# zhen6618/EPRecon

Measured on AMD Instinct MI355X. Metric: fragments_per_sec, higher is better.
Workload: dtype f32

## Files before the change

### eprecon_amd/_lib.py

```python
import ctypes
import os

import numpy as np
import torch

_HERE = os.path.dirname(os.path.abspath(__file__))
LIB_PATH = os.environ.get("EPRECON_LIB_PATH") or os.path.join(_HERE, "libeprecon_hip.so")

_c = ctypes
_vp, _i, _i64, _f, _sz = _c.c_void_p, _c.c_int, _c.c_int64, _c.c_float, _c.c_size_t

SIGNATURES = {
    "eprecon_abi_version": (_i, []),
    "eprecon_build_arch": (_c.c_char_p, []),
    "eprecon_count_mailbox": (_i, []),
    "eprecon_mailbox_acquire": (_i, [_i, _vp]),
    "eprecon_mailbox_wait": (_i, [_vp, _i64, _vp]),
    "eprecon_mailbox_release": (_i, [_vp]),
    "eprecon_mailbox_free_slots": (_i, []),
    "eprecon_back_project_workspace_bytes": (_sz, [_i64, _i, _i, _i, _i, _i, _i]),
    "eprecon_back_project_async": (_i, [_vp, _i64, _vp, _i, _f, _vp, _i, _vp, _i, _i, _i, _i, _i, _i,
                                        _vp, _vp, _vp, _vp, _vp, _vp, _vp, _vp, _sz, _vp]),
    "eprecon_back_project_call_async": (_i, [_vp, _vp]),
    "eprecon_back_project_call": (_i, [_vp, _i, _vp, _vp]),
    "eprecon_back_project_prepare_levels_async": (_i, [_vp, _i, _vp]),
    "eprecon_back_project_workspace_maps_offset": (_sz, [_i64, _i]),
    "eprecon_bp_levels": (_i, []),
    "eprecon_init_glue": (_i, []),
    "eprecon_profile_gather_kernel": (_c.c_char_p, []),
    "eprecon_hash_capacity": (_c.c_uint32, [_i64]),
    "eprecon_hash_table_bytes": (_sz, [_c.c_uint32]),
    "eprecon_hash_build_async": (_i, [_vp, _i64, _i, _vp, _c.c_uint32, _vp]),
    "eprecon_hash_build_dn_async": (_i, [_vp, _i64, _vp, _i, _vp, _c.c_uint32, _vp]),
    "eprecon_hash_query_async": (_i, [_vp, _c.c_uint32, _vp, _i64, _i, _vp, _vp]),
    "eprecon_hash_status": (_i, [_vp, _vp]),
    "eprecon_unique_workspace_bytes": (_sz, [_i64]),
    "eprecon_unique_coords_async": (_i, [_vp, _i64, _i, _vp, _c.c_uint32, _vp, _vp, _vp, _vp, _sz, _vp]),
    "eprecon_unique_coords_dn_async": (_i, [_vp, _i64, _vp, _i, _vp, _c.c_uint32, _vp, _vp, _vp, _vp, _sz, _vp]),
    "eprecon_unique_hierarchy_dn_async": (_i, [_vp, _i64, _vp, _i, _vp, _vp, _vp, _vp, _vp, _vp, _sz, _vp]),
    "eprecon_point_quantize_dn_async": (_i, [_vp, _i64, _vp, _f, _vp, _vp, _vp]),
    "eprecon_spvcnn_points_dn_async": (_i, [_vp, _i64, _vp, _i, _i, _vp, _i, _f, _vp, _f, _vp, _vp, _vp, _vp, _vp, _vp]),
    "eprecon_gru_stage_capacity": (_i64, [_vp, _i64, _i]),
# ... 244 lines not shown


class ViewsDesc(ctypes.Structure):
    _fields_ = [("src", (ctypes.c_void_p * 16) * 3), ("dst", ctypes.c_void_p * 3), ("channels", ctypes.c_int32 * 3),
                ("hw", ctypes.c_int32 * 3), ("levels", ctypes.c_int32), ("n_views", ctypes.c_int32)]


class BpCall(ctypes.Structure):
    _fields_ = [("coords", ctypes.c_void_p), ("n", ctypes.c_int64), ("origin", ctypes.c_void_p), ("batch", ctypes.c_int32),
                ("voxel_size", ctypes.c_float), ("feats", ctypes.c_void_p), ("feats_layout", ctypes.c_int32),
                ("krcam", ctypes.c_void_p), ("n_views", ctypes.c_int32), ("channels", ctypes.c_int32), ("height", ctypes.c_int32),
                ("width", ctypes.c_int32), ("min_view", ctypes.c_int32), ("mode", ctypes.c_int32), ("count", ctypes.c_void_p),
                ("n_valid_dev", ctypes.c_void_p), ("workspace", ctypes.c_void_p), ("workspace_bytes", ctypes.c_size_t),
                ("phase", ctypes.c_int32), ("out_feats", ctypes.c_void_p), ("out_mean", ctypes.c_void_p),
                ("out_coords", ctypes.c_void_p), ("out_grid", ctypes.c_void_p), ("out_mask", ctypes.c_void_p),
                ("rank", ctypes.c_void_p), ("counts_host", ctypes.c_void_p), ("counts_seq", ctypes.c_uint32)]


class MailboxSlot(ctypes.Structure):
    _fields_ = [("payload_dev", ctypes.c_void_p), ("payload_host", ctypes.c_void_p), ("seq", ctypes.c_uint32),
                ("index", ctypes.c_int32), ("words", ctypes.c_int32), ("armed", ctypes.c_int32)]


class AdamSegment(ctypes.Structure):
    _fields_ = [("param", ctypes.c_void_p), ("grad", ctypes.c_void_p), ("exp_avg", ctypes.c_void_p),
                ("exp_avg_sq", ctypes.c_void_p)]


class AdamChunk(ctypes.Structure):
    _fields_ = [("segment", ctypes.c_int32), ("start", ctypes.c_int32), ("count", ctypes.c_int32), ("flags", ctypes.c_int32)]

# ... 302 lines not shown
```

### eprecon_amd/back_project.py

```python
import ctypes

import torch
import torch.nn as nn

from . import _lib

MODE_MEAN, MODE_MEAN_DEPTH, MODE_VARIANCE = 0, 1, 2
LAYOUT_NCHW, LAYOUT_NHWC = 0, 1


def mark_dense(coords, dims, interval, batch=1):
    coords._eprecon_dense = (tuple(int(d) for d in dims), int(interval), int(batch))
    return coords


def dense_rank_buffer(coords, dims, interval):
    tag = getattr(coords, "_eprecon_dense", None)
    want = (tuple(int(d) for d in dims), int(interval), 1)
    if tag != want or not coords.is_cuda or coords.shape[0] != want[0][0] * want[0][1] * want[0][2]:
        return None
    if not _lib.load().eprecon_init_glue():
        return None
    return torch.empty(coords.shape[0] + 1, dtype=torch.int32, device=coords.device)

# ... 126 lines not shown
        self._slots = [hd.mailbox for hd in handles]
        self._read = None if all(m is not None for m in self._slots) else _lib.PinnedRead(handles[0].n_valid_all)

    def results(self):
        if self._host is None and self._read is None:
            _lib.count_host_read()
            self._host = [None] * (self._offsets[-1] + 1 + self._pends[-1]._batch)
            for m, p, o in zip(self._slots, self._pends, self._offsets):
                self._host[o:o + 1 + p._batch] = m.wait()
        elif self._host is None:
            self._host = self._read.result()
        return [p.result_from(self._host[o:o + 1 + p._batch]) for p, o in zip(self._pends, self._offsets)]


def prepare_levels_async(levels, stream=None):
    lib = _lib.load()
    if not 1 <= len(levels) <= 4:
        raise _lib.EpreconError("prepare_levels_async takes one to four levels")
    dev = levels[0][3].device
    rows = []
    for lv in levels:
        coords, origin, voxel_size, feats, krcam, min_view = lv[:6]
        mode = lv[6] if len(lv) > 6 else MODE_MEAN
        shape = tuple(int(x) for x in feats.shape)
        feats_c, layout = _prep_feats(feats)
        inputs = None if coords is None else _prep_inputs(coords, origin, krcam, shape[0], shape[1], dev)
        rows.append((shape, feats_c, layout, inputs, float(voxel_size), int(min_view), mode))
    n_valid_all = torch.empty((sum(1 + r[0][1] for r in rows if r[3] is not None),), dtype=torch.int32, device=dev)
    descs = (_lib.BpCall * len(rows))()
    listed = [r for r in rows if r[3] is not None]
# ... 9 lines not shown
        _call(inputs, feats_c, shape, layout, voxel_size, min_view, mode, {"count": count}, n_valid_dev, ws, d=d)
        nhwc = feats_c
        if layout == LAYOUT_NCHW:
            o = lib.eprecon_back_project_workspace_maps_offset(n, b)
            nhwc = ws[o:o + 4 * v * b * c * h * w].view(torch.float32).view(v, b, h, w, c).permute(0, 1, 4, 2, 3)
        if inputs is None:
            handles.append(PreparedMaps(nhwc, (ws, feats_c), stream))
            continue
        mb = next(slots)
        if mb is not None:
            d.counts_host, d.counts_seq = mb.payload_dev, mb.seq
        hd = CountedBackProject(shape, inputs + (voxel_size, min_view, mode), d, count, n_valid_dev, ws, stream, mailbox=mb)
        hd.nhwc, hd.feats, hd.n_valid_all, hd.n_valid_off = nhwc, feats_c, n_valid_all, off
        handles.append(hd)
        off += 1 + b

    def queue():
        _lib.check(lib.eprecon_back_project_prepare_levels_async(ctypes.byref(descs), len(rows), _lib.current_stream()),
                   "eprecon_back_project_prepare_levels_async")
        for hd in handles:
            if getattr(hd, "mailbox", None) is not None:
                hd.mailbox.queued(hd.n_valid_dev)
    if stream is None:
        queue()
    else:
        stream.wait_stream(torch.cuda.current_stream(dev))
        with torch.cuda.stream(stream):
            queue()
    return handles


def run_async(coords, origin, voxel_size, feats, krcam, min_view, mode=MODE_MEAN, min_valid_per_batch=1,
              want_grid=False, want_mean=False, hold_read=False, extra_words=0, rank_out=None, counted=None):
    lib = _lib.load()
    dev = feats.device
    shape = v, b, c, h, w = tuple(feats.shape)
    inputs = _prep_inputs(coords, origin, krcam, v, b, dev)
    n = coords.shape[0]
    feats_c, layout = _prep_feats(feats)
    t = _alloc_outputs(n, v, c, mode, want_grid, want_mean, dev, count=None if counted is None else counted.count)
    if counted is not None:
        assert layout == LAYOUT_NHWC and counted.shape == shape and not extra_words
        assert counted.inputs[3:] == (float(voxel_size), int(min_view), mode) and counted.count.shape[0] == n
        inputs, n_valid_dev, ws = counted.inputs[:3], counted.n_valid_dev, counted.ws
        if counted.stream is not None:
            torch.cuda.current_stream(dev).wait_stream(counted.stream)
    else:
        n_valid_dev = torch.empty((1 + b + int(extra_words),), dtype=torch.int32, device=dev)
        ws = _lib.workspace(lib.eprecon_back_project_workspace_bytes(n, b, v, c, h, w, layout), dev)
    mb, early = (counted.mailbox, counted.early) if counted is not None else (None, False)
    if mb is None and not hold_read and n > 0:
        mb = _lib.mailbox_read(1 + b)
    if counted is not None:
        call = _lib.BpCall.from_buffer_copy(counted.call)
        call.feats, call.feats_layout = _lib.ptr(feats_c), layout
        _set_outputs(call, t, rank_out, phase=2)
    else:
        call = _call(inputs, feats_c, shape, layout, voxel_size, min_view, mode, t, n_valid_dev, ws, rank_out)
    call.counts_host, call.counts_seq = (mb.payload_dev, mb.seq) if mb is not None and not early else (None, 0)
    _lib.check(lib.eprecon_back_project_call_async(ctypes.byref(call), _lib.current_stream()), "eprecon_back_project_call_async")
    if mb is not None and not early:
        mb.queued(n_valid_dev)
    read = None if hold_read else mb if mb is not None else _lib.PinnedRead(n_valid_dev[:1 + b])
    t["_keep"] = (*inputs, feats_c, n_valid_dev, ws if counted is not None else None)
    pend = PendingBackProject(t, n, v, c, b, int(min_valid_per_batch), read, want_grid, want_mean)
    pend.n_valid_dev, pend.coords_all = n_valid_dev, t["coords"]
    return pend


def run(coords, origin, voxel_size, feats, krcam, min_view, mode=MODE_MEAN, min_valid_per_batch=1,
        want_grid=False, want_mean=False, rank_out=None):
    lib = _lib.load()
    dev = feats.device
    shape = v, b, c, h, w = tuple(feats.shape)
# ... 92 lines not shown
```

### eprecon_amd/csrc/back_project.hip

```cpp
#include <stdlib.h>

#include "back_project_gather.hpp"

namespace {

constexpr int kFoldCapDefault = 6144;

size_t gather_lds_bytes(bool mlp, int vox, int V, int B)
{
    const size_t nP = ((size_t)V * B * 12 + 3) & ~(size_t)3;
    return (size_t)vox * V * (mlp ? 12 : 8) + nP * 4 + (size_t)vox * (mlp ? 3 : 5) * 4 + (size_t)(256 / kWave) * 4 * 3;
}

template <int VOX, int MODE>
int launch_gather(const BpParams &p, bool mlp, hipStream_t st)
{
    const size_t lds = gather_lds_bytes(mlp, VOX, p.V, p.batch);
    const dim3 grid(p.ntile), block(256);
    if (p.C % 4 != 0) {
        hipLaunchKernelGGL((bp_gather_kernel<VOX, MODE, 1, 0>), grid, block, lds, st, p);
    } else {
        pick<6, 8, 10, 20, 0>(p.C / 4, [&](auto qt) {
            constexpr int QT = decltype(qt)::value;
            if (mlp) hipLaunchKernelGGL((bp_gather_mlp_kernel<VOX, MODE, QT, 1>), grid, block, lds, st, p);
            else hipLaunchKernelGGL((bp_gather_kernel<VOX, MODE, 4, QT>), grid, block, lds, st, p);
            return 0;
        });
    }
    EP_LAUNCH_CHECK();
    return EPRECON_OK;
}

struct BpCarve {
    size_t rows, maps, end;
// ... 24 lines not shown
    if (!a.workspace || (!a.feats && !(listed && !rows && nhwc))) return EPRECON_ERR_ARG;
    if (listed && (!a.origin || !a.krcam || !a.n_valid_dev)) return EPRECON_ERR_ARG;
    if (listed && a.n > 0 && (!a.coords || !a.count || (rows && (!a.out_feats || !a.out_coords)))) return EPRECON_ERR_ARG;
    if (a.counts_host && (!listed || a.n == 0 || a.counts_seq == 0 || 1 + a.batch > EPRECON_MAILBOX_WORDS)) return EPRECON_ERR_ARG;
    if ((size_t)a.n_views * a.batch * 12 * sizeof(float) > 32 * 1024) return EPRECON_ERR_UNSUPPORTED;
    if (a.workspace_bytes < eprecon_back_project_workspace_bytes(a.n, a.batch, a.n_views, a.channels, a.height, a.width,
                                                                 a.feats_layout))
        return EPRECON_ERR_WORKSPACE;
    if ((size_t)a.n_views * a.batch * a.channels * a.height * a.width > 0x7fffffffull) return EPRECON_ERR_UNSUPPORTED;
    return EPRECON_OK;
}

struct BpPlan {
    bool nchw, chain4, clear_in_relayout, mlp;
    int vox, ntile, nblk_count;
    size_t lds_relayout, lds_count;
    int32_t *tile_sums, *blk_batch;
    float *nhwc;
    BpParams p;
};

BpPlan bp_plan(const eprecon_bp_call &a)
{
    BpPlan pl;
    const int64_t n = a.n;
    pl.nchw = a.feats_layout == EPRECON_LAYOUT_NCHW;
    int fold_cap = kFoldCapDefault;
    if (const char *e = getenv("EPRECON_BP_FOLD"); e && e[0]) {
        const long v = strtol(e, nullptr, 10);
        fold_cap = v <= 0 ? 0 : (v > 0x7fffffffL ? 0x7fffffff : (int)v);
// ... 16 lines not shown
    p.min_view = a.min_view; p.out_feats = a.out_feats; p.out_mean = a.out_mean; p.out_coords = a.out_coords;
    p.count = a.count; p.out_grid = a.out_grid; p.out_mask = a.out_mask; p.n_valid_dev = a.n_valid_dev;
    p.block_offsets = pl.tile_sums;
    p.rank = a.phase == EPRECON_BP_COUNT ? nullptr : a.rank;
    p.counts_host = a.counts_host; p.counts_seq = a.counts_seq;
    p.xcd_slabs = ep::switch_off("EPRECON_BP_XCD_SLABS") ? 0 : 1;
    pl.mlp = p.C % 4 == 0 && p.Cs % 4 == 0 && p.V <= 32 && (size_t)p.V * p.batch * p.H * p.W * p.Cs * 4 < 0x7fff0000ull &&
             gather_lds_bytes(true, 256, p.V, p.batch) <= dynamic_lds_limit();

    pl.vox = n >= 512 * 1024 ? 256 : (n >= 48 * 1024 ? 64 : 16);
    if (pl.vox == 256 && !pl.mlp && gather_lds_bytes(false, 256, a.n_views, a.batch) > dynamic_lds_limit()) pl.vox = 64;
    pl.ntile = (int)ep::ceil_div(n, pl.vox);
    pl.nblk_count = (int)ep::ceil_div(n, 256);
    p.fold = (!pl.chain4 && pl.ntile <= fold_cap) ? 1 : 0;
    p.ntile = pl.ntile; p.blk_batch = pl.blk_batch; p.nblk_count = pl.nblk_count;
    return pl;
}

int bp_clear_counters(const eprecon_bp_call &a, hipStream_t st)
{
    EP_HIP_CHECK(hipMemsetAsync(a.n_valid_dev, 0, sizeof(int32_t) * (size_t)(1 + a.batch), st));
    return EPRECON_OK;
}

int bp_launch_scan(const BpPlan &pl, hipStream_t st, bool write_back = true)
{
    hipLaunchKernelGGL(bp_scan_kernel, dim3(1), dim3(1024), 0, st, pl.tile_sums, pl.ntile, pl.p.n_valid_dev,
                       (const int32_t *)pl.blk_batch, pl.nblk_count, pl.p.batch, write_back ? 1 : 0, pl.p.counts_host,
                       pl.p.counts_seq);
    EP_LAUNCH_CHECK();
// ... 33 lines not shown
    EP_LAUNCH_CHECK();
    if (!p.fold) return bp_launch_scan(pl, st);
    return early_publish && p.counts_host ? bp_launch_scan(pl, st, false) : EPRECON_OK;
}

template <int VOX>
int bp_queue_gather(const eprecon_bp_call &a, const BpPlan &pl, hipStream_t st)
{
    if (a.n == 0) {
        if (a.rank) EP_HIP_CHECK(hipMemsetAsync(a.rank, 0, sizeof(int32_t), st));
        return EPRECON_OK;
    }
    int rc = ep::profile_bracket_begin(st);
    if (rc != EPRECON_OK) return rc;
    rc = pick<EPRECON_BP_MEAN, EPRECON_BP_MEAN_DEPTH, EPRECON_BP_VARIANCE>(
        a.mode, [&](auto mode) { return launch_gather<VOX, decltype(mode)::value>(pl.p, pl.mlp, st); });
    if (rc != EPRECON_OK) return rc;
    rc = ep::profile_bracket_end(st, pl.mlp ? "bp_gather_mlp_kernel" : "bp_gather_kernel");
    if (rc != EPRECON_OK) return rc;
    if (a.mode == EPRECON_BP_MEAN_DEPTH) {
        hipLaunchKernelGGL(bp_depth_norm_kernel, dim3(a.batch), dim3(1024), 0, st, a.out_feats, a.channels + 1, a.n_valid_dev);
        EP_LAUNCH_CHECK();
    }
    return EPRECON_OK;
}

int bp_queue(const eprecon_bp_call &a, const BpPlan &pl, hipStream_t st, bool early_publish = false)
{
    return pick<256, 64, 16>(pl.vox, [&](auto vox) {
        constexpr int VOX = decltype(vox)::value;
        const int rc = a.phase != EPRECON_BP_GATHER ? bp_queue_count<VOX>(a, pl, st, early_publish) : EPRECON_OK;
// ... 72 lines not shown
        d.end = cursor;
    }
    if (cursor > 0) {
        hipLaunchKernelGGL(bp_prepare_levels_kernel, dim3((unsigned)cursor), dim3(256), lds, st, t);
        EP_LAUNCH_CHECK();
    }
    for (int l = 0; l < n_levels; ++l) {
        if (listed[l] && calls[l].n > 0 && !plans[l].p.fold) {
            const int rc = bp_launch_scan(plans[l], st);
            if (rc != EPRECON_OK) return rc;
        }
    }
    return EPRECON_OK;
}

}

extern "C" {

size_t eprecon_back_project_workspace_bytes(int64_t n, int batch, int n_views, int channels,
                                            int height, int width, int feats_layout)
{
    const size_t map_bytes =
        feats_layout == EPRECON_LAYOUT_NCHW ? (size_t)n_views * batch * channels * height * width * sizeof(float) : 0;
    return bp_carve(n > 0 ? n : 1, batch > 0 ? batch : 1, map_bytes).end + 256;
}

size_t eprecon_back_project_workspace_maps_offset(int64_t n, int batch) { return bp_carve(n, batch, 0).maps; }

int eprecon_nchw_to_nhwc_async(const float *in, float *out, int maps, int channels, int hw,
                               void *stream)
{
    if (!in || !out || maps <= 0 || channels <= 0 || hw <= 0) return EPRECON_ERR_ARG;
// ... 59 lines not shown
```

### eprecon_amd/csrc/back_project_gather.hpp

```cpp
#pragma once
#include "back_project_count.hpp"

namespace {


struct TileBase {
    int base, n_valid;
};

__device__ __forceinline__ bool tile_base_all(const BpParams &p, int lb)
{
    return p.out_grid != nullptr || p.out_mask != nullptr || lb == p.ntile - 1;
}

__device__ __forceinline__ void tile_base_partials(const BpParams &p, int lb, int *sFold)
{
    constexpr int BLOCK = 256;
    const int tid = threadIdx.x, lane = tid & (kWave - 1), wid = tid / kWave;
    const int end = tile_base_all(p, lb) ? p.ntile : lb;
    int acc = 0, tot = 0;
#pragma unroll 4
    for (int t = tid; t < end; t += BLOCK) {
        const int x = p.block_offsets[t];
        tot += x;
// ... 37 lines not shown
                if (tid == 0) {
                    int t = 0;
                    for (int w = 0; w < NW; ++w) t += sFold[w];
                    p.n_valid_dev[1 + b] = t;
                }
            }
        }
        if (tid == 0 && p.counts_host) mailbox_publish(p.counts_host, p.counts_seq, p.n_valid_dev, 1 + p.batch);
    }
    return r;
}

__device__ __forceinline__ void gather_rank_store(const BpParams &p, int lb, int e, bool mine, bool valid, int orow)
{
    if (mine) p.rank[e] = valid ? orow : -1;
    if (lb == (int)gridDim.x - 1 && threadIdx.x == 0) p.rank[p.n] = 0;
}


template <int VOX, int MODE, int VEC, int QT>
__global__ __launch_bounds__(256) void bp_gather_kernel(BpParams p)
{
    extern __shared__ __attribute__((aligned(16))) char smem[];
    constexpr int BLOCK = 256;
    float2 *sPix = reinterpret_cast<float2 *>(smem);
    float *sP = reinterpret_cast<float *>(sPix + VOX * p.V);
    const int nP = (p.V * p.batch * 12 + 3) & ~3;
    uint32_t *sVis = reinterpret_cast<uint32_t *>(sP + nP);
    float *sDen = reinterpret_cast<float *>(sVis + VOX);
    int *sBatch = reinterpret_cast<int *>(sDen + VOX);
    int *sSlot = sBatch + VOX;
// ... 136 lines not shown
#pragma unroll
        for (int u = 0; u < U; ++u) {
            const float wx1 = wxy[u].x, wy1 = wxy[u].y;
            const float wx0 = 1.0f - wx1, wy0 = 1.0f - wy1;
            const float w00 = wx0 * wy0, w10 = wx1 * wy0, w01 = wx0 * wy1, w11 = wx1 * wy1;
            float4 r;
#define EP_TAP(k) fmaf(__uint_as_float(d[u].k), w11, fmaf(__uint_as_float(c[u].k), w01, fmaf(__uint_as_float(b[u].k), w10, __uint_as_float(a[u].k) * w00)))
            r.x = EP_TAP(x); r.y = EP_TAP(y); r.z = EP_TAP(z); r.w = EP_TAP(w);
#undef EP_TAP
            if (on[u]) f(r);
        }
    }
}

template <int VOX, int MODE, int QT, int U>
__global__ __launch_bounds__(256) void bp_gather_mlp_kernel(BpParams p)
{
    extern __shared__ __attribute__((aligned(16))) char smem[];
    constexpr int BLOCK = 256;
    constexpr int VPT = BLOCK / VOX;
    float2 *sWxy = reinterpret_cast<float2 *>(smem);
    int *sOff = reinterpret_cast<int *>(sWxy + VOX * p.V);
    float *sP = reinterpret_cast<float *>(sOff + VOX * p.V);
    const int nP = (p.V * p.batch * 12 + 3) & ~3;
    uint32_t *sVis = reinterpret_cast<uint32_t *>(sP + nP);
    int *sSlot = reinterpret_cast<int *>(sVis + VOX);
    int *sOut = sSlot + VOX;
    int *sWave = sOut + VOX;
    int *sFold = sWave + BLOCK / kWave;

    const int tid = threadIdx.x;
    const int lb = p.xcd_slabs ? xcd_remap(blockIdx.x, gridDim.x) : (int)blockIdx.x;
    stage_matrices(sP, p.krcam, p.V * p.batch, tid, BLOCK);
    if (VPT > 1 && tid < VOX) sVis[tid] = 0;
    if (p.fold) tile_base_partials(p, lb, sFold);
    __syncthreads();

    const float wm1 = (float)(p.W - 1), hm1 = (float)(p.H - 1);
    const float kx = 2.0f / wm1, ky = 2.0f / hm1;
    const int map_elems = p.H * p.W * p.Cs;
    const int vx = tid % VOX;
    const int e = lb * VOX + vx;
    int4 c = make_int4(-1, 0, 0, 0);
    if (e < p.n) c = reinterpret_cast<const int4 *>(p.coords)[e];
    const bool in_batch = c.x >= 0 && c.x < p.batch;
    uint32_t vis = 0;
    if (in_batch) {
        float X, Y, Z;
// ... 67 lines not shown
            visit_visible_samples<U>(rsrc, offRow, wxyRow, vm, q * 16, s10, s01, s11, [&](const float4 &f) {
                const float dx = f.x - mean.x, dy = f.y - mean.y, dz = f.z - mean.z, dw = f.w - mean.w;
                sq.x = fmaf(dx, dx, sq.x); sq.y = fmaf(dy, dy, sq.y); sq.z = fmaf(dz, dz, sq.z); sq.w = fmaf(dw, dw, sq.w);
            });
            *reinterpret_cast<float4 *>(dst) = make_float4(__fdiv_rn(sq.x, den), __fdiv_rn(sq.y, den),
                                                           __fdiv_rn(sq.z, den), __fdiv_rn(sq.w, den));
            if (p.out_mean) *reinterpret_cast<float4 *>(p.out_mean + (size_t)orow * p.C + q * 4) = mean;
        } else if (MODE == EPRECON_BP_MEAN_DEPTH) {
            dst[0] = mean.x; dst[1] = mean.y; dst[2] = mean.z; dst[3] = mean.w;
        } else {
            *reinterpret_cast<float4 *>(dst) = mean;
        }
    }
}

__global__ __launch_bounds__(1024) void bp_depth_norm_kernel(float *out_feats, int cout,
                                                             const int32_t *n_valid_dev)
{
    __shared__ float sRed[1024 / kWave];
    const int b = blockIdx.x, tid = threadIdx.x, lane = tid & (kWave - 1), wid = tid / kWave;
    int start = 0;
    for (int k = 0; k < b; ++k) start += n_valid_dev[1 + k];
    const int len = n_valid_dev[1 + b];
    float *d = out_feats + (size_t)start * cout + (cout - 1);

    auto block_sum = [&](float x) -> float {
#pragma unroll
        for (int s = kWave / 2; s > 0; s >>= 1) x += __shfl_xor(x, s);
        __syncthreads();
        if (lane == 0) sRed[wid] = x;
// ... 27 lines not shown
```

### eprecon_amd/csrc/common.hpp

```cpp
#pragma once

#include <hip/hip_runtime.h>
#include <stdint.h>
#include <stdlib.h>

#include <type_traits>

#include "../../include/eprecon_hip.h"

#define EP_HIP_CHECK(expr)                                            \
    do {                                                              \
        hipError_t e_ = (expr);                                       \
        if (e_ != hipSuccess) return EPRECON_ERR_HIP_BASE - (int)e_;  \
    } while (0)
#define EP_LAUNCH_CHECK() EP_HIP_CHECK(hipGetLastError())

namespace ep {

constexpr int kWave = 64;
constexpr int kXcd = 8;

static inline size_t align_up(size_t x, size_t a) { return (x + a - 1) / a * a; }
static inline int64_t ceil_div(int64_t a, int64_t b) { return (a + b - 1) / b; }

inline bool switch_off(const char *name)
{
    const char *e = getenv(name);
    return e && e[0] == '0';
}
inline bool switch_on(const char *name)
{
    const char *e = getenv(name);
    return e && e[0] == '1';
}

// ... 6 lines not shown

static inline size_t dynamic_lds_limit()
{
    static const size_t limit = [] {
        int dev = 0, v = 0;
        if (hipGetDevice(&dev) != hipSuccess ||
            hipDeviceGetAttribute(&v, hipDeviceAttributeMaxSharedMemoryPerBlock, dev) != hipSuccess || v <= 0)
            v = 64 * 1024;
        return (size_t)(v < 64 * 1024 ? v : 64 * 1024);
    }();
    return limit;
}

__device__ __forceinline__ int xcd_remap(int hw_bid, int nblk)
{
    const int q = nblk / kXcd, r = nblk % kXcd;
    const int xcd = hw_bid % kXcd, k = hw_bid / kXcd;
    const int start = xcd < r ? xcd * (q + 1) : r * (q + 1) + (xcd - r) * q;
    return start + k;
}

__device__ __forceinline__ void mailbox_publish(int32_t *payload, uint32_t seq, const int32_t *values, int n)
{
    for (int i = 0; i < n; ++i) payload[i] = values[i];
    __threadfence_system();
    __hip_atomic_store(reinterpret_cast<uint32_t *>(payload) - 1, seq, __ATOMIC_RELEASE, __HIP_MEMORY_SCOPE_SYSTEM);
}

template <int BLOCK>
__device__ __forceinline__ int block_exclusive_rank(bool pred, int *wave_counts, int &block_total)
{
    const unsigned long long m = __ballot(pred);
    const int lane = threadIdx.x & (kWave - 1);
    const int wid = threadIdx.x / kWave;
// ... 36 lines not shown
```

### eprecon_amd/fragment_step.py

```python
import os

import torch

from . import _lib
from . import back_project as BP
from . import grid_ops as GO
from . import synthetic as S
from .config import CH_IMG, CH_INIT_DOWN, N_VIEWS
from .occupancy_initialization import Occupancy_Initialization

LEVELS = [("bp24", 2, 4, 2), ("bp48", 1, 2, 0), ("bp96", 0, 1, 0)]


class Cfg2Step:
    def __init__(self, seed=0, device=None, height=480, width=640, n_vox=(96, 96, 96)):
        self.device = device or torch.device("cuda")
        self.seed = seed
        self.window = S.make_window(seed=seed, width=width, height=height, n_vox=n_vox)
        self.shapes = S.pyramid_shapes(height, width)
        dev = self.device
        t = lambda a: torch.from_numpy(a).to(dev)
        self.origin = t(self.window["vol_origin_partial"][None].copy())
        self.voxel_size = self.window["voxel_size"]
        self.krcam = [t(self.window["proj_matrices"][:, l][:, None].copy()) for l in range(3)]
        self.feats = [t(S.make_features(1000 * seed + 10 + l, N_VIEWS, self.shapes[l])) for l in range(3)]
        f1 = [t(S.make_features(1000 * seed + 20 + l, N_VIEWS, self.shapes[l])) for l in range(3)]
        self.features_init = [[f1[l][v] for l in range(3)] for v in range(N_VIEWS)]
        self.coords = {iv: BP.mark_dense(t(S.dense_coords(n_vox, iv)), [n // iv for n in n_vox], iv) for iv in (4, 2, 1)}
        self.shape_init = tuple(n // 2 for n in n_vox)
        torch.manual_seed(1234)
        self.init_net = Occupancy_Initialization(CH_IMG, CH_INIT_DOWN, N_VIEWS).to(dev)
        self.init_net.train()
        self.last = {}
        self.defer_reads = False
        self._inflight = None
        self.levels_inside = True
        self.profile_dominant = False
        self.bp_side_stream = False
        self._bp_stream = None
        self.levels_beside_2d = False

    @torch.no_grad()
    def run(self):
        issued = self._issue()
        if not self.defer_reads:
            return self._finish(issued)
        prev, self._inflight = self._inflight, issued
        return self._finish(prev) if prev is not None else {}

    def flush(self):
        if self._inflight is not None:
            prev, self._inflight = self._inflight, None
            return self._finish(prev)
        return self.last

# ... 2 lines not shown
        if select is not None:
            out["stage0_coords"], _ = select.result()
        for name in pending:
            if name == "_levels":
                names, read = pending[name]
                out.update(zip(names, read.results()))
            else:
                out[name] = pending[name].result()
        self.last = out
        return out

    def _issue(self):
        out = {}
        pending = {}
        main = torch.cuda.current_stream(self.device)
        side = self._bp_stream if self.bp_side_stream else main

        one_launch = self.levels_inside and not self.bp_side_stream and bool(_lib.load().eprecon_bp_levels())

        def prepare_levels(stream):
            return BP.prepare_levels_async(
                [(self.coords[interval], self.origin, self.voxel_size, self.feats[lvl], self.krcam[lvl], mv)
                 for _, lvl, interval, mv in LEVELS], stream=stream)
        beside = self.levels_beside_2d or os.environ.get("EPRECON_BP_LEVELS_BESIDE", "0") == "1"
        early = prepare_levels(_lib.side_stream(self.device, _lib.SIDE_SETUP)) if one_launch and beside else None

        def queue_levels():
            if one_launch:
                handles = early if early is not None else prepare_levels(None)
                pends = []
                for (name, lvl, interval, mv), hd in zip(LEVELS, handles):
                    if self.profile_dominant and name == "bp96":
                        _lib.load().eprecon_profile_enable(2)
                    pends.append(BP.run_async(self.coords[interval], self.origin, self.voxel_size, hd.nhwc, self.krcam[lvl], mv,
                                              hold_read=True, counted=hd))
                pending["_levels"] = ([l[0] for l in LEVELS], BP.PendingLevels(pends, handles))
                return
            if side is not main:
                side.wait_stream(main)
            with torch.cuda.stream(side):
                for name, lvl, interval, mv in LEVELS:
                    if self.profile_dominant and name == "bp96":
                        _lib.load().eprecon_profile_enable(2)
                    pending[name] = BP.run_async(self.coords[interval], self.origin, self.voxel_size, self.feats[lvl],
                                                 self.krcam[lvl], mv)

        if not self.levels_inside:
            queue_levels()
        init = self.init_net(self.coords[2], self.origin, self.voxel_size, self.features_init,
                             self.krcam[1], self.shape_init, 1, 2, between=queue_levels if self.levels_inside else None)
        out["init"] = init
        select = None
        if init is not None:
            select = GO.init_select_async(init[0], init[1], 1, dim=self.shape_init[0] // 2, cell=4, dense=self.init_net.dense_map)
        if side is not main:
            main.wait_stream(side)
        return out, pending, select

    def dominant_kernel_ms(self, lib):
        return float(lib.eprecon_profile_gather_ms())

    def dominant_kernel_bytes(self):
        c, h, w = self.shapes[0]
        n = self.coords[1].shape[0]
        nv = self.last["bp96"]["n_valid"] if self.last.get("bp96") else n
        return 16 * n + 4 * N_VIEWS * c * h * w + nv * (4 * c + 16)

    def dominant_kernel_l1_bandwidth(self, launch_ms):
        if not launch_ms:
            return None
        c = self.shapes[0][0]
# ... 299 lines not shown
```

### include/eprecon_hip.h

```cpp
#ifndef EPRECON_HIP_H
#define EPRECON_HIP_H

#include <stddef.h>
#include <stdint.h>

#ifdef __cplusplus
extern "C" {
#endif

#define EPRECON_OK 0
#define EPRECON_EMPTY 1
#define EPRECON_ERR_ARG (-1)
#define EPRECON_ERR_WORKSPACE (-2)
#define EPRECON_ERR_UNSUPPORTED (-3)
#define EPRECON_ERR_TIMEOUT (-4)
#define EPRECON_ERR_HIP_BASE (-1000)

#define EPRECON_ABI_VERSION 2
int eprecon_abi_version(void);
const char *eprecon_build_arch(void);

#define EPRECON_MAILBOX_WORDS 15
typedef struct eprecon_mailbox_slot {
    int32_t *payload_dev;
// ... 31 lines not shown
    int32_t feats_layout;
    const float *krcam;
    int32_t n_views, channels, height, width, min_view, mode;
    float *count;
    int32_t *n_valid_dev;
    void *workspace;
    size_t workspace_bytes;
    int32_t phase;
    float *out_feats, *out_mean;
    int32_t *out_coords;
    float *out_grid;
    uint8_t *out_mask;
    int32_t *rank;
    int32_t *counts_host;
    uint32_t counts_seq;
} eprecon_bp_call;

int eprecon_back_project_call_async(const eprecon_bp_call *call, void *stream);

int eprecon_back_project_call(const eprecon_bp_call *call, int min_valid_per_batch, int32_t *n_valid_host, void *stream);

int eprecon_back_project_async(const int32_t *coords, int64_t n, const float *origin, int batch,
                               float voxel_size, const float *feats, int feats_layout,
                               const float *krcam, int n_views, int channels, int height,
                               int width, int min_view, int mode, float *out_feats,
                               float *out_mean, int32_t *out_coords, float *count,
                               float *out_grid, uint8_t *out_mask, int32_t *n_valid_dev,
                               void *workspace, size_t workspace_bytes, void *stream);

int eprecon_back_project_prepare_levels_async(const eprecon_bp_call *levels, int n_levels, void *stream);
size_t eprecon_back_project_workspace_maps_offset(int64_t n, int batch);
int eprecon_bp_levels(void);

int eprecon_init_glue(void);

int eprecon_profile_enable(int on);
float eprecon_profile_gather_ms(void);
const char *eprecon_profile_gather_kernel(void);

int eprecon_profile_conv_arm(int kvol, int cin, int cout, int64_t min_rows);
float eprecon_profile_conv_ms(int64_t *rows_out, const char **kernel_out);
int64_t eprecon_profile_conv_pairs(void);
int64_t eprecon_profile_conv_executed_pairs(void);
const char *eprecon_profile_last_conv_kernel(void);
int eprecon_profile_mark_async(int id, void *stream);

int eprecon_nchw_to_nhwc_async(const float *in, float *out, int maps, int channels, int hw,
// ... 538 lines not shown
```

Measured before the change: 842.7.

## Fuse level prepare and gathers into one native call, add persistent gather kernel

Adds a native entry point that prepares all back-projection levels and queues their gather kernels in one call, which replaces the per-level Python run_async calls. Adds an optional persistent (resident) gather kernel that stages the camera matrices once per block and walks several tiles in XCD-aware slabs. It is controlled by an env var that defaults to off. The fragment step now uses the fused path by default, and can optionally run it on the side stream when resident mode is on. This mainly removes host launch overhead, at the cost of extra code paths and descriptor plumbing.

```diff
diff --git a/eprecon_amd/_lib.py b/eprecon_amd/_lib.py
--- a/eprecon_amd/_lib.py
+++ b/eprecon_amd/_lib.py
@@ -26,6 +26,9 @@
     "eprecon_back_project_prepare_levels_async": (_i, [_vp, _i, _vp]),
     "eprecon_back_project_workspace_maps_offset": (_sz, [_i64, _i]),
     "eprecon_bp_levels": (_i, []),
+    "eprecon_back_project_levels_async": (_i, [_vp, _i, _vp, _i]),
+    "eprecon_bp_resident": (_i, []),
+    "eprecon_bp_resident_launches": (_i64, []),
     "eprecon_init_glue": (_i, []),
     "eprecon_profile_gather_kernel": (_c.c_char_p, []),
     "eprecon_hash_capacity": (_c.c_uint32, [_i64]),
@@ -300,7 +303,8 @@
                 ("n_valid_dev", ctypes.c_void_p), ("workspace", ctypes.c_void_p), ("workspace_bytes", ctypes.c_size_t),
                 ("phase", ctypes.c_int32), ("out_feats", ctypes.c_void_p), ("out_mean", ctypes.c_void_p),
                 ("out_coords", ctypes.c_void_p), ("out_grid", ctypes.c_void_p), ("out_mask", ctypes.c_void_p),
-                ("rank", ctypes.c_void_p), ("counts_host", ctypes.c_void_p), ("counts_seq", ctypes.c_uint32)]
+                ("rank", ctypes.c_void_p), ("counts_host", ctypes.c_void_p), ("counts_seq", ctypes.c_uint32),
+                ("resident_groups", ctypes.c_int32)]
 
 
 class MailboxSlot(ctypes.Structure):
diff --git a/eprecon_amd/back_project.py b/eprecon_amd/back_project.py
--- a/eprecon_amd/back_project.py
+++ b/eprecon_amd/back_project.py
@@ -164,6 +164,56 @@
 
 
 def prepare_levels_async(levels, stream=None):
+    descs, handles = _level_descriptors(levels, stream)
+
+    def queue():
+        _lib.check(_lib.load().eprecon_back_project_prepare_levels_async(ctypes.byref(descs), len(descs), _lib.current_stream()),
+                   "eprecon_back_project_prepare_levels_async")
+    _queue_levels(queue, handles, stream, levels[0][3].device)
+    return handles
+
+
+def levels_async(levels, stream=None, profile_level=-1, resident_groups=0):
+    descs, handles = _level_descriptors(levels, stream)
+    pends, listed = [], []
+    for d, hd in zip(descs, handles):
+        if isinstance(hd, PreparedMaps):
+            continue
+        v, b, c, h, w = hd.shape
+        mode, n = hd.inputs[5], hd.count.shape[0]
+        t = _alloc_outputs(n, v, c, mode, False, False, hd.count.device, count=hd.count)
+        _set_outputs(d, t)
+        d.resident_groups = int(resident_groups)
+        t["_keep"] = (*hd.inputs[:3], hd.feats, hd.n_valid_dev, hd.ws)
+        pend = PendingBackProject(t, n, v, c, b, 1, None, False, False)
+        pend.n_valid_dev, pend.coords_all = hd.n_valid_dev, t["coords"]
+        pends.append(pend)
+        listed.append(hd)
+
+    def queue():
+        _lib.check(_lib.load().eprecon_back_project_levels_async(ctypes.byref(descs), len(descs), _lib.current_stream(),
+                                                                 int(profile_level)), "eprecon_back_project_levels_async")
+    _queue_levels(queue, handles, stream, levels[0][3].device)
+    read = PendingLevels(pends, listed)
+    read.handles = handles
+    return read
+
+
+def _queue_levels(queue, handles, stream, dev):
+    def go():
+        queue()
+        for hd in handles:
+            if getattr(hd, "mailbox", None) is not None:
+                hd.mailbox.queued(hd.n_valid_dev)
+    if stream is None:
+        go()
+    else:
+        stream.wait_stream(torch.cuda.current_stream(dev))
+        with torch.cuda.stream(stream):
+            go()
+
+
+def _level_descriptors(levels, stream):
     lib = _lib.load()
     if not 1 <= len(levels) <= 4:
         raise _lib.EpreconError("prepare_levels_async takes one to four levels")
@@ -203,24 +253,11 @@
         hd.nhwc, hd.feats, hd.n_valid_all, hd.n_valid_off = nhwc, feats_c, n_valid_all, off
         handles.append(hd)
         off += 1 + b
-
-    def queue():
-        _lib.check(lib.eprecon_back_project_prepare_levels_async(ctypes.byref(descs), len(rows), _lib.current_stream()),
-                   "eprecon_back_project_prepare_levels_async")
-        for hd in handles:
-            if getattr(hd, "mailbox", None) is not None:
-                hd.mailbox.queued(hd.n_valid_dev)
-    if stream is None:
-        queue()
-    else:
-        stream.wait_stream(torch.cuda.current_stream(dev))
-        with torch.cuda.stream(stream):
-            queue()
-    return handles
+    return descs, handles
 
 
 def run_async(coords, origin, voxel_size, feats, krcam, min_view, mode=MODE_MEAN, min_valid_per_batch=1,
-              want_grid=False, want_mean=False, hold_read=False, extra_words=0, rank_out=None, counted=None):
+              want_grid=False, want_mean=False, hold_read=False, extra_words=0, rank_out=None, counted=None, resident_groups=0):
     lib = _lib.load()
     dev = feats.device
     shape = v, b, c, h, w = tuple(feats.shape)
@@ -247,6 +284,7 @@
     else:
         call = _call(inputs, feats_c, shape, layout, voxel_size, min_view, mode, t, n_valid_dev, ws, rank_out)
     call.counts_host, call.counts_seq = (mb.payload_dev, mb.seq) if mb is not None and not early else (None, 0)
+    call.resident_groups = int(resident_groups)
     _lib.check(lib.eprecon_back_project_call_async(ctypes.byref(call), _lib.current_stream()), "eprecon_back_project_call_async")
     if mb is not None and not early:
         mb.queued(n_valid_dev)
diff --git a/eprecon_amd/csrc/back_project.hip b/eprecon_amd/csrc/back_project.hip
--- a/eprecon_amd/csrc/back_project.hip
+++ b/eprecon_amd/csrc/back_project.hip
@@ -1,4 +1,6 @@
 #include <stdlib.h>
+
+#include <atomic>
 
 #include "back_project_gather.hpp"
 
@@ -12,12 +14,45 @@
     return (size_t)vox * V * (mlp ? 12 : 8) + nP * 4 + (size_t)vox * (mlp ? 3 : 5) * 4 + (size_t)(256 / kWave) * 4 * 3;
 }
 
+constexpr int kResidentDefault = 0;
+const int g_resident_k = [] {
+    const char *e = getenv("EPRECON_BP_RESIDENT");
+    if (!e || !e[0]) return kResidentDefault;
+    const long v = strtol(e, nullptr, 10);
+    return v <= 0 ? 0 : (v > 16 ? 16 : (int)v);
+}();
+
+std::atomic<int64_t> g_resident_launches{0};
+
+int compute_units()
+{
+    static const int n = [] {
+        int dev = 0, v = 0;
+        if (hipGetDevice(&dev) != hipSuccess ||
+            hipDeviceGetAttribute(&v, hipDeviceAttributeMultiprocessorCount, dev) != hipSuccess || v <= 0)
+            v = 256;
+        return v;
+    }();
+    return n;
+}
+
+template <int VOX>
+constexpr int kResidentChannels = VOX == 256 ? 24 : (VOX == 64 ? 40 : 80);
+
 template <int VOX, int MODE>
-int launch_gather(const BpParams &p, bool mlp, hipStream_t st)
+int launch_gather(const BpParams &p, bool mlp, int groups, hipStream_t st)
 {
     const size_t lds = gather_lds_bytes(mlp, VOX, p.V, p.batch);
     const dim3 grid(p.ntile), block(256);
-    if (p.C % 4 != 0) {
+    if (groups > 0) {
+        if constexpr (MODE == EPRECON_BP_MEAN) {
+            constexpr int QT = kResidentChannels<VOX> / 4;
+            hipLaunchKernelGGL((bp_gather_mlp_resident_kernel<VOX, MODE, QT, 1>), dim3(groups), block, lds, st, p);
+            g_resident_launches.fetch_add(1, std::memory_order_relaxed);
+        } else {
+            return EPRECON_ERR_ARG;
+        }
+    } else if (p.C % 4 != 0) {
         hipLaunchKernelGGL((bp_gather_kernel<VOX, MODE, 1, 0>), grid, block, lds, st, p);
     } else {
         pick<6, 8, 10, 20, 0>(p.C / 4, [&](auto qt) {
@@ -72,6 +107,7 @@
 struct BpPlan {
     bool nchw, chain4, clear_in_relayout, mlp;
     int vox, ntile, nblk_count;
+    int groups;
     size_t lds_relayout, lds_count;
     int32_t *tile_sums, *blk_batch;
     float *nhwc;
@@ -118,6 +154,12 @@
     pl.nblk_count = (int)ep::ceil_div(n, 256);
     p.fold = (!pl.chain4 && pl.ntile <= fold_cap) ? 1 : 0;
     p.ntile = pl.ntile; p.blk_batch = pl.blk_batch; p.nblk_count = pl.nblk_count;
+    pl.groups = 0;
+    const int c_res = pl.vox == 256 ? kResidentChannels<256> : (pl.vox == 64 ? kResidentChannels<64> : kResidentChannels<16>);
+    if (pl.mlp && a.mode == EPRECON_BP_MEAN && p.C == c_res && a.resident_groups >= 0) {
+        const int64_t g = a.resident_groups > 0 ? a.resident_groups : (int64_t)g_resident_k * compute_units();
+        pl.groups = (int)(g < pl.ntile ? g : pl.ntile);
+    }
     return pl;
 }
 
@@ -181,7 +223,7 @@
     int rc = ep::profile_bracket_begin(st);
     if (rc != EPRECON_OK) return rc;
     rc = pick<EPRECON_BP_MEAN, EPRECON_BP_MEAN_DEPTH, EPRECON_BP_VARIANCE>(
-        a.mode, [&](auto mode) { return launch_gather<VOX, decltype(mode)::value>(pl.p, pl.mlp, st); });
+        a.mode, [&](auto mode) { return launch_gather<VOX, decltype(mode)::value>(pl.p, pl.mlp, pl.groups, st); });
     if (rc != EPRECON_OK) return rc;
     rc = ep::profile_bracket_end(st, pl.mlp ? "bp_gather_mlp_kernel" : "bp_gather_kernel");
     if (rc != EPRECON_OK) return rc;
@@ -284,9 +326,43 @@
     return EPRECON_OK;
 }
 
+int bp_levels_impl(const eprecon_bp_call *levels, int n_levels, hipStream_t st, int profile_level)
+{
+    if (!levels || n_levels <= 0 || n_levels > kMaxLevels || profile_level >= n_levels) return EPRECON_ERR_ARG;
+    eprecon_bp_call gathers[kMaxLevels];
+    for (int l = 0; l < n_levels; ++l) {
+        if (!levels[l].coords) continue;
+        eprecon_bp_call &g = gathers[l];
+        g = levels[l];
+        g.phase = EPRECON_BP_GATHER;
+        if (g.feats_layout == EPRECON_LAYOUT_NCHW) {
+            if (g.n < 0 || g.batch <= 0 || !g.workspace) return EPRECON_ERR_ARG;
+            g.feats = reinterpret_cast<const float *>(reinterpret_cast<const char *>(g.workspace) + bp_carve(g.n, g.batch, 0).maps);
+            g.feats_layout = EPRECON_LAYOUT_NHWC;
+        }
+        const int rc = bp_validate(g, kBpGatherHalf);
+        if (rc != EPRECON_OK) return rc;
+    }
+    int rc = bp_prepare_levels_impl(levels, n_levels, st);
+    for (int l = 0; l < n_levels && rc == EPRECON_OK; ++l) {
+        if (!levels[l].coords) continue;
+        if (l == profile_level) rc = eprecon_profile_enable(2);
+        if (rc == EPRECON_OK) rc = bp_queue(gathers[l], bp_plan(gathers[l]), st);
+    }
+    return rc;
+}
+
 }
 
 extern "C" {
+
+int eprecon_bp_resident(void) { return g_resident_k; }
+int64_t eprecon_bp_resident_launches(void) { return g_resident_launches.load(std::memory_order_relaxed); }
+
+int eprecon_back_project_levels_async(const eprecon_bp_call *levels, int n_levels, void *stream, int profile_level)
+{
+    return bp_levels_impl(levels, n_levels, (hipStream_t)stream, profile_level);
+}
 
 size_t eprecon_back_project_workspace_bytes(int64_t n, int batch, int n_views, int channels,
                                             int height, int width, int feats_layout)
diff --git a/eprecon_amd/csrc/back_project_gather.hpp b/eprecon_amd/csrc/back_project_gather.hpp
--- a/eprecon_amd/csrc/back_project_gather.hpp
+++ b/eprecon_amd/csrc/back_project_gather.hpp
@@ -75,7 +75,7 @@
 __device__ __forceinline__ void gather_rank_store(const BpParams &p, int lb, int e, bool mine, bool valid, int orow)
 {
     if (mine) p.rank[e] = valid ? orow : -1;
-    if (lb == (int)gridDim.x - 1 && threadIdx.x == 0) p.rank[p.n] = 0;
+    if (lb == p.ntile - 1 && threadIdx.x == 0) p.rank[p.n] = 0;
 }
 
 
@@ -242,9 +242,8 @@
 }
 
 template <int VOX, int MODE, int QT, int U>
-__global__ __launch_bounds__(256) void bp_gather_mlp_kernel(BpParams p)
-{
-    extern __shared__ __attribute__((aligned(16))) char smem[];
+__device__ __forceinline__ void gather_mlp_tile(const BpParams &p, int lb, char *smem)
+{
     constexpr int BLOCK = 256;
     constexpr int VPT = BLOCK / VOX;
     float2 *sWxy = reinterpret_cast<float2 *>(smem);
@@ -258,8 +257,6 @@
     int *sFold = sWave + BLOCK / kWave;
 
     const int tid = threadIdx.x;
-    const int lb = p.xcd_slabs ? xcd_remap(blockIdx.x, gridDim.x) : (int)blockIdx.x;
-    stage_matrices(sP, p.krcam, p.V * p.batch, tid, BLOCK);
     if (VPT > 1 && tid < VOX) sVis[tid] = 0;
     if (p.fold) tile_base_partials(p, lb, sFold);
     __syncthreads();
@@ -357,6 +354,34 @@
     }
 }
 
+template <int VOX>
+__device__ __forceinline__ float *gather_mlp_matrices(const BpParams &p, char *smem)
+{
+    return reinterpret_cast<float *>(reinterpret_cast<int *>(reinterpret_cast<float2 *>(smem) + VOX * p.V) + VOX * p.V);
+}
+
+template <int VOX, int MODE, int QT, int U>
+__global__ __launch_bounds__(256) void bp_gather_mlp_kernel(BpParams p)
+{
+    extern __shared__ __attribute__((aligned(16))) char smem[];
+    const int lb = p.xcd_slabs ? xcd_remap(blockIdx.x, gridDim.x) : (int)blockIdx.x;
+    stage_matrices(gather_mlp_matrices<VOX>(p, smem), p.krcam, p.V * p.batch, threadIdx.x, 256);
+    gather_mlp_tile<VOX, MODE, QT, U>(p, lb, smem);
+}
+
+template <int VOX, int MODE, int QT, int U>
+__global__ __launch_bounds__(256) void bp_gather_mlp_resident_kernel(BpParams p)
+{
+    extern __shared__ __attribute__((aligned(16))) char smem[];
+    stage_matrices(gather_mlp_matrices<VOX>(p, smem), p.krcam, p.V * p.batch, threadIdx.x, 256);
+    const TileWalk w = tile_walk((int)blockIdx.x, (int)gridDim.x, p.ntile, p.xcd_slabs != 0);
+#pragma nounroll
+    for (int lb = w.first; lb < w.end; lb += w.step) {
+        gather_mlp_tile<VOX, MODE, QT, U>(p, lb, smem);
+        __syncthreads();
+    }
+}
+
 __global__ __launch_bounds__(1024) void bp_depth_norm_kernel(float *out_feats, int cout,
                                                              const int32_t *n_valid_dev)
 {
diff --git a/eprecon_amd/csrc/common.hpp b/eprecon_amd/csrc/common.hpp
--- a/eprecon_amd/csrc/common.hpp
+++ b/eprecon_amd/csrc/common.hpp
@@ -7,6 +7,7 @@
 #include <type_traits>
 
 #include "../../include/eprecon_hip.h"
+#include "xcd_walk.hpp"
 
 #define EP_HIP_CHECK(expr)                                            \
     do {                                                              \
@@ -18,7 +19,6 @@
 namespace ep {
 
 constexpr int kWave = 64;
-constexpr int kXcd = 8;
 
 static inline size_t align_up(size_t x, size_t a) { return (x + a - 1) / a * a; }
 static inline int64_t ceil_div(int64_t a, int64_t b) { return (a + b - 1) / b; }
@@ -55,10 +55,7 @@
 
 __device__ __forceinline__ int xcd_remap(int hw_bid, int nblk)
 {
-    const int q = nblk / kXcd, r = nblk % kXcd;
-    const int xcd = hw_bid % kXcd, k = hw_bid / kXcd;
-    const int start = xcd < r ? xcd * (q + 1) : r * (q + 1) + (xcd - r) * q;
-    return start + k;
+    return xcd_slab(hw_bid % kXcd, nblk).start + hw_bid / kXcd;
 }
 
 __device__ __forceinline__ void mailbox_publish(int32_t *payload, uint32_t seq, const int32_t *values, int n)
diff --git a/eprecon_amd/csrc/xcd_walk.hpp b/eprecon_amd/csrc/xcd_walk.hpp
--- /dev/null
+++ b/eprecon_amd/csrc/xcd_walk.hpp
@@ -0,0 +1,36 @@
+#pragma once
+
+#if defined(__HIPCC__) || defined(__CUDACC__)
+#define EP_HOST_DEVICE __host__ __device__ __forceinline__
+#else
+#define EP_HOST_DEVICE inline
+#endif
+
+namespace ep {
+
+constexpr int kXcd = 8;
+
+struct Slab {
+    int start, size;
+};
+EP_HOST_DEVICE Slab xcd_slab(int s, int nblk, int nslab = kXcd)
+{
+    const int q = nblk / nslab, r = nblk % nslab;
+    return {s < r ? s * (q + 1) : r * (q + 1) + (s - r) * q, s < r ? q + 1 : q};
+}
+
+struct TileWalk {
+    int first, step, end;
+};
+
+EP_HOST_DEVICE TileWalk tile_walk(int b, int groups, int ntile, bool slabs)
+{
+    if (!slabs) return {b, groups, ntile};
+    const int nslab = groups < kXcd ? groups : kXcd;
+    const int s = b % nslab, j = b / nslab;
+    const int mates = groups / nslab + (s < groups % nslab ? 1 : 0);
+    const Slab sl = xcd_slab(s, ntile, nslab);
+    return {sl.start + j, mates, sl.start + sl.size};
+}
+
+}
diff --git a/eprecon_amd/fragment_step.py b/eprecon_amd/fragment_step.py
--- a/eprecon_amd/fragment_step.py
+++ b/eprecon_amd/fragment_step.py
@@ -37,8 +37,9 @@
         self.levels_inside = True
         self.profile_dominant = False
         self.bp_side_stream = False
-        self._bp_stream = None
         self.levels_beside_2d = False
+        self.levels_on_side = None
+        self.resident_groups = 0
 
     @torch.no_grad()
     def run(self):
@@ -71,36 +72,42 @@
         out = {}
         pending = {}
         main = torch.cuda.current_stream(self.device)
-        side = self._bp_stream if self.bp_side_stream else main
-
-        one_launch = self.levels_inside and not self.bp_side_stream and bool(_lib.load().eprecon_bp_levels())
-
-        def prepare_levels(stream):
-            return BP.prepare_levels_async(
-                [(self.coords[interval], self.origin, self.voxel_size, self.feats[lvl], self.krcam[lvl], mv)
-                 for _, lvl, interval, mv in LEVELS], stream=stream)
+        setup = _lib.side_stream(self.device, _lib.SIDE_SETUP)
+        lib = _lib.load()
+
+        one_launch = self.levels_inside and not self.bp_side_stream and bool(lib.eprecon_bp_levels())
+        level_args = [(self.coords[interval], self.origin, self.voxel_size, self.feats[lvl], self.krcam[lvl], mv)
+                      for _, lvl, interval, mv in LEVELS]
         beside = self.levels_beside_2d or os.environ.get("EPRECON_BP_LEVELS_BESIDE", "0") == "1"
-        early = prepare_levels(_lib.side_stream(self.device, _lib.SIDE_SETUP)) if one_launch and beside else None
+        early = BP.prepare_levels_async(level_args, stream=setup) if one_launch and beside else None
+        on_side = one_launch and early is None and (bool(lib.eprecon_bp_resident()) if self.levels_on_side is None
+                                                    else bool(self.levels_on_side))
+        joined = on_side or self.bp_side_stream
+
+        def bracket(name):
+            if self.profile_dominant and name == "bp96":
+                lib.eprecon_profile_enable(2)
 
         def queue_levels():
-            if one_launch:
-                handles = early if early is not None else prepare_levels(None)
+            if one_launch and early is None:
+                read = BP.levels_async(level_args, stream=setup if on_side else None,
+                                       profile_level=2 if self.profile_dominant else -1, resident_groups=self.resident_groups)
+                pending["_levels"] = ([l[0] for l in LEVELS], read)
+            elif one_launch:
                 pends = []
-                for (name, lvl, interval, mv), hd in zip(LEVELS, handles):
-                    if self.profile_dominant and name == "bp96":
-                        _lib.load().eprecon_profile_enable(2)
+                for (name, lvl, interval, mv), hd in zip(LEVELS, early):
+                    bracket(name)
                     pends.append(BP.run_async(self.coords[interval], self.origin, self.voxel_size, hd.nhwc, self.krcam[lvl], mv,
                                               hold_read=True, counted=hd))
-                pending["_levels"] = ([l[0] for l in LEVELS], BP.PendingLevels(pends, handles))
-                return
-            if side is not main:
-                side.wait_stream(main)
-            with torch.cuda.stream(side):
-                for name, lvl, interval, mv in LEVELS:
-                    if self.profile_dominant and name == "bp96":
-                        _lib.load().eprecon_profile_enable(2)
-                    pending[name] = BP.run_async(self.coords[interval], self.origin, self.voxel_size, self.feats[lvl],
-                                                 self.krcam[lvl], mv)
+                pending["_levels"] = ([l[0] for l in LEVELS], BP.PendingLevels(pends, early))
+            else:
+                if self.bp_side_stream:
+                    setup.wait_stream(main)
+                with torch.cuda.stream(setup if self.bp_side_stream else main):
+                    for name, lvl, interval, mv in LEVELS:
+                        bracket(name)
+                        pending[name] = BP.run_async(self.coords[interval], self.origin, self.voxel_size, self.feats[lvl],
+                                                     self.krcam[lvl], mv)
 
         if not self.levels_inside:
             queue_levels()
@@ -110,8 +117,8 @@
         select = None
         if init is not None:
             select = GO.init_select_async(init[0], init[1], 1, dim=self.shape_init[0] // 2, cell=4, dense=self.init_net.dense_map)
-        if side is not main:
-            main.wait_stream(side)
+        if joined:
+            main.wait_stream(setup)
         return out, pending, select
 
     def dominant_kernel_ms(self, lib):
diff --git a/include/eprecon_hip.h b/include/eprecon_hip.h
--- a/include/eprecon_hip.h
+++ b/include/eprecon_hip.h
@@ -69,6 +69,7 @@
     int32_t *rank;
     int32_t *counts_host;
     uint32_t counts_seq;
+    int32_t resident_groups;
 } eprecon_bp_call;
 
 int eprecon_back_project_call_async(const eprecon_bp_call *call, void *stream);
@@ -86,6 +87,11 @@
 int eprecon_back_project_prepare_levels_async(const eprecon_bp_call *levels, int n_levels, void *stream);
 size_t eprecon_back_project_workspace_maps_offset(int64_t n, int batch);
 int eprecon_bp_levels(void);
+
+int eprecon_back_project_levels_async(const eprecon_bp_call *levels, int n_levels, void *stream, int profile_level);
+
+int eprecon_bp_resident(void);
+int64_t eprecon_bp_resident_launches(void);
 
 int eprecon_init_glue(void);
 
```

After: 841.0. About the same (-0.2%).
